# js43o/HifiDiff

Hardware: AMD Instinct MI355X
Metric: faces/sec (whole node), 16→128 1000-step reverse diffusion, batch 64 (higher is better)
Workload: dtype bf16

## Files before the change

hifidiff_amd/_lib.py:

```python
import ctypes
import os
import subprocess

import torch

_HERE = os.path.dirname(os.path.abspath(__file__))
LIB_PATH = os.path.join(_HERE, "libhifidiff_hip.so")
UNITS = [os.path.join(_HERE, "csrc", f) for f in ("hd_lib.hip", "hd_aux.hip", "hd_stages.hip", "hd_stages_rows.hip", "hd_strip.hip", "hd_dispatch_ln.hip", "hd_dispatch_lnface.hip", "hd_dispatch_bf16.hip", "hd_dispatch_misc.hip", "hd_lpips.hip", "hd_photo.hip", "hd_image.hip")]
SOURCES = UNITS + [os.path.join(_HERE, "csrc", f) for f in ("hd_gemm.hpp", "hd_dispatch.hpp", "hd_kernels.hpp", "hd_chain.hpp", "hd_conv.hpp", "hd_cr.hpp", "hd_vae.hpp", "hd_internal.hpp", "hd_faceset.hpp", "hd_stage_api.hpp", "hd_xcd.hpp", "hd_xcd2.hpp", "hd_face.hpp", "hd_strip.hpp", "hd_wide.hpp", "hd_end.hpp", "hd_color.hpp", "hd_metrics.hpp", "hd_lpips.hpp", "hd_photo.hpp", "hd_args.hpp", "hd_bicubic.hpp")]
HEADER = os.path.join(os.path.dirname(_HERE), "include", "hifidiff_hip.h")


def unit_deps(unit):
    import re
    seen, todo = [], [unit]
    while todo:
        f = os.path.normpath(todo.pop())
        if f in seen or not os.path.exists(f):
            continue
        seen.append(f)
        with open(f) as fh:
            for inc in re.findall(r'^\s*#include\s+"([^"]+)"', fh.read(), flags=re.M):
                todo.append(os.path.join(os.path.dirname(f), inc))
    return seen
# ... 33 lines not shown
class GemmNote(ctypes.Structure):
    _fields_ = [(n, ctypes.c_int32) for n in ("op_info", "family", "rows", "pair", "wk", "cpw", "nt", "wide_form", "threads", "grid_x", "grid_y")]


GEMM_DRY_RUN = 1


class ConvDesc(ctypes.Structure):
    _fields_ = [(n, ctypes.c_int32) for n in ("M", "C", "side", "face0", "stats_np", "stats_cnt", "film_off", "film_face_stride")] + \
               [("T1_elems", ctypes.c_int64)] + \
               [(n, ctypes.c_void_p) for n in ("X", "out", "out16", "stats_out", "stats_in", "film", "G", "pooled", "pooled16", "T1")]


class ConvNote(ctypes.Structure):
    _fields_ = [(n, ctypes.c_int32) for n in ("form", "centre_only", "C", "side", "bm", "mt", "ks", "nt", "strip", "depth", "faces_per_wg", "threads",
                                              "grid_x", "grid_y", "remap", "hint", "dw_path")] + [("gemm", GemmNote)]


CONV_HCA, CONV_DOWN, CONV_DWGATE = 0, 1, 2


def build(force=False, verbose=False):
    if not force and os.path.exists(LIB_PATH):
        newest = max(os.path.getmtime(p) for p in SOURCES + [HEADER])
        if os.path.getmtime(LIB_PATH) >= newest:
            return LIB_PATH
    hipcc = os.environ.get("HIPCC", "/opt/rocm/bin/hipcc")
    flags = ["--offload-arch=gfx950", "-O3", "-std=c++17", "-fPIC", "-Wno-unused-result", "-Wno-unused-function"]
    objdir = os.path.join(_HERE, "csrc", "build")
    os.makedirs(objdir, exist_ok=True)
    objs = [os.path.join(objdir, os.path.splitext(os.path.basename(u))[0] + ".o") for u in UNITS]
# ... 110 lines not shown
```

hifidiff_amd/csrc/hd_conv.hpp:

```cpp
#pragma once
#include "hd_gemm.hpp"
#ifndef HD_CONV_DEPTH
#define HD_CONV_DEPTH 8
#endif
#ifndef HD_CONV_NT_MINC
#define HD_CONV_NT_MINC 1024
#endif

#define HD_CONV_XCD_REMAP(C, grid_x, grid_y) ((C) >= 1024 && ((grid_y) & 7) == 0 && (grid_x) > 1)

namespace hd {

struct ConvP {
    int M;
    const unsigned short* X;
    const uint4* W;
    const float* bias;
    float* out;
    unsigned short* out16;
};

template <int C_, int S_, int BM_, int MT_, int KS_, int DEPTH_ = 8, bool STRIP_ = false, int NT_ = 1>
struct ConvCfg {
    static constexpr int C = C_, S = S_, HW = S_ * S_, BM = BM_, MT = MT_, KS = KS_, NT = NT_;
    static constexpr bool STRIP = STRIP_;
    static constexpr int RG = BM / (32 * MT);
    static constexpr int WAVES = RG * KS, THREADS = 64 * WAVES;
    static constexpr int NP = STRIP ? BM + 2 * S : (BM > HW ? BM : HW);
    static constexpr int ROWB = C * 2 + 16;
    static constexpr int KSTEPS = 9 * C / 16;
    static constexpr int SPT = C / 16, CPW = SPT / KS;
    static constexpr int NSTEP = 9 * CPW;
    static constexpr int XIN = (NP + 1) * ROWB;
    static constexpr int RED = KS > 1 ? KS * BM * 32 * 4 : 0;
// ... 1 lines not shown
    static constexpr int DEPTH = DEPTH_;
    static constexpr int OCC = (NT_ > 1 && C_ == 512) ? 4 : 1;
    static_assert(WAVES == 8 || WAVES == 4, "4 or 8 waves");
    static_assert(NSTEP >= DEPTH, "prefetch ring longer than the loop");
    static_assert(SPT % KS == 0 && BM % (32 * MT) == 0, "shape");
    static_assert((HW >= BM && HW % BM == 0) || (BM % HW == 0), "row tiles are whole faces or a face is whole row tiles");
    static_assert(!STRIP || (BM % S == 0 && HW % BM == 0 && HW > BM), "a strip is whole image rows of one face");
};

template <class K>
__global__ __launch_bounds__((K::THREADS), (K::OCC)) void hca_conv_kernel(const ConvP p) {
    extern __shared__ __attribute__((aligned(16))) char smem[];
    constexpr int C = K::C, S = K::S, HW = K::HW, MT = K::MT, KS = K::KS;
    const int tid = threadIdx.x, lane = tid & 63, wave = tid >> 6;
    const int rg = wave / KS, ksl = wave - rg * KS;
    int bx = blockIdx.x, tile = blockIdx.y;
    if (HD_CONV_XCD_REMAP(K::C, gridDim.x, gridDim.y)) {
        const int lin = blockIdx.y * gridDim.x + blockIdx.x, j = lin >> 3;
        bx = j % (int)gridDim.x;
        tile = (j / (int)gridDim.x) * 8 + (lin & 7);
    }
    const int row0 = bx * K::BM;
    const int pix0 = K::STRIP ? row0 - S : (row0 / K::NP) * K::NP;
    uint4 bq[K::DEPTH][K::NT];
    const uint4* Wl = p.W + ((size_t)tile * K::NT * K::KSTEPS + ksl * K::CPW) * 64 + lane;
#define HD_CONV_B(n, t) (K::C >= HD_CONV_NT_MINC ? nt_load_u4(&Wl[(size_t)((t) * K::KSTEPS + ((n) / K::CPW) * K::SPT + ((n) % K::CPW)) * 64]) \
                                      : Wl[(size_t)((t) * K::KSTEPS + ((n) / K::CPW) * K::SPT + ((n) % K::CPW)) * 64])
#pragma unroll
    for (int d = 0; d < K::DEPTH; ++d)
#pragma unroll
// ... 35 lines not shown
            for (int t = 0; t < 9; ++t) {
                const int yy = y + t / 3 - 1, xx = x + t % 3 - 1;
                const bool in = yy >= 0 && yy < S && xx >= 0 && xx < S;
                src_off[mt][t] = (in ? (sbase + yy * S + xx) : K::NP) * K::ROWB + h * 16;
            }
        }
    }
    f32x16_t acc[MT][K::NT];
#pragma unroll
    for (int mt = 0; mt < MT; ++mt)
#pragma unroll
        for (int t = 0; t < K::NT; ++t)
#pragma unroll
            for (int i = 0; i < 16; ++i) acc[mt][t][i] = 0.f;
    __syncthreads();

    const int cbase = ksl * K::CPW * 32;
#pragma unroll
    for (int n = 0; n < K::NSTEP; ++n) {
        const int tap = n / K::CPW, j = n % K::CPW;
        bf16x8_t a[MT];
#pragma unroll
        for (int mt = 0; mt < MT; ++mt) a[mt] = *reinterpret_cast<const bf16x8_t*>(smem + src_off[mt][tap] + cbase + j * 32);
#pragma unroll
        for (int t = 0; t < K::NT; ++t) {
            const bf16x8_t b = __builtin_bit_cast(bf16x8_t, bq[n % K::DEPTH][t]);
#pragma unroll
            for (int mt = 0; mt < MT; ++mt) acc[mt][t] = __builtin_amdgcn_mfma_f32_32x32x16_bf16(a[mt], b, acc[mt][t], 0, 0, 0);
        }
        if (n + K::DEPTH < K::NSTEP) {
#pragma unroll
            for (int t = 0; t < K::NT; ++t) bq[n % K::DEPTH][t] = HD_CONV_B(n + K::DEPTH, t);
            asm volatile("" ::: "memory");
        }
    }
#undef HD_CONV_B

    if constexpr (KS > 1) __syncthreads();
#pragma unroll
    for (int t = 0; t < K::NT; ++t) {
        const int col = (tile * K::NT + t) * 32 + (lane & 31);
        const float bias = p.bias[col];
        if constexpr (KS > 1) {
            float* red = reinterpret_cast<float*>(smem);
            if (t > 0) __syncthreads();
#pragma unroll
            for (int mt = 0; mt < MT; ++mt)
#pragma unroll
                for (int i = 0; i < 16; ++i) {
                    const int r = (rg * MT + mt) * 32 + (i & 3) + 8 * (i >> 2) + 4 * (lane >> 5);
                    red[(ksl * K::BM + r) * 32 + (lane & 31)] = acc[mt][t][i];
                }
            __syncthreads();
            for (int e = tid; e < K::BM * 32; e += K::THREADS) {
                float v = bias;
#pragma unroll
                for (int s = 0; s < KS; ++s) v += red[s * K::BM * 32 + e];
                v = fmaxf(v, 0.f);
                const int row = row0 + (e >> 5);
                if (row < p.M) {
                    p.out[(size_t)row * C + col] = v;
                    if (p.out16) p.out16[(size_t)row * C + col] = f32_to_bf16_bits(v);
                }
            }
        } else {
#pragma unroll
            for (int mt = 0; mt < MT; ++mt)
#pragma unroll
                for (int i = 0; i < 16; ++i) {
                    const int row = row0 + (rg * MT + mt) * 32 + (i & 3) + 8 * (i >> 2) + 4 * (lane >> 5);
                    const float v = fmaxf(acc[mt][t][i] + bias, 0.f);
                    if (row < p.M) {
                        p.out[(size_t)row * C + col] = v;
                        if (p.out16) p.out16[(size_t)row * C + col] = f32_to_bf16_bits(v);
                    }
                }
        }
    }
}

struct ConvLaunchNote { int C, S, BM, MT, KS, NT, strip, depth, threads, grid_x, grid_y, remap; };
inline thread_local ConvLaunchNote g_conv_note = {};

template <class K>
inline hipError_t launch_hca_conv(const ConvP& p, hipStream_t s) {
    if (K::SMEM > 65536) {
        static std::atomic<unsigned long long> granted{0};
        { const hipError_t e = grant_dynamic_lds(reinterpret_cast<const void*>(&hca_conv_kernel<K>), K::SMEM, granted); if (e != hipSuccess) return e; }
    }
    const dim3 grid((p.M + K::BM - 1) / K::BM, K::C / (32 * K::NT));
    g_conv_note = ConvLaunchNote{K::C, K::S, K::BM, K::MT, K::KS, K::NT, K::STRIP ? 1 : 0, K::DEPTH, K::THREADS, (int)grid.x, (int)grid.y,
                                 HD_CONV_XCD_REMAP(K::C, grid.x, grid.y) ? 1 : 0};
    hipLaunchKernelGGL((hca_conv_kernel<K>), grid, dim3(K::THREADS), K::SMEM, s, p);
    return hipGetLastError();
}

typedef ConvCfg<128, 16, 256, 2, 2, HD_CONV_DEPTH> ConvL0;
typedef ConvCfg<256, 8, 128, 2, 4, HD_CONV_DEPTH> ConvL1;
typedef ConvCfg<512, 4, 64, 2, 8, HD_CONV_DEPTH> ConvL2;
typedef ConvCfg<1024, 2, 32, 1, 8, 16> ConvL3;
#ifndef HD_CONV_L2X32_NT
#define HD_CONV_L2X32_NT 1
#endif
typedef ConvCfg<128, 32, 256, 2, 2, 4, true, 4> ConvL0x32;
typedef ConvCfg<256, 16, 256, 2, 2, 8, false, 2> ConvL1x32;
typedef ConvCfg<512, 8, 64, 2, 8, (HD_CONV_L2X32_NT > 1 ? 4 : 8), false, HD_CONV_L2X32_NT> ConvL2x32;
typedef ConvCfg<1024, 4, 64, 2, 8, 8, false, 2> ConvL3x32;
typedef ConvCfg<2048, 2, 32, 1, 8, 8, false, 2> ConvL4x32;

}
```

hifidiff_amd/csrc/hd_internal.hpp:

```cpp
#pragma once
#include <hip/hip_runtime.h>

#include <cmath>
#include <cstdio>
#include <cstring>
#include <functional>
#include <map>
#include <memory>
#include <string>
#include <unordered_map>
#include <vector>

#include "../../include/hifidiff_hip.h"
#include "hd_chain.hpp"
#include "hd_conv.hpp"
#include "hd_cr.hpp"
#include "hd_dispatch.hpp"
#include "hd_gemm.hpp"
#include "hd_kernels.hpp"
#include "hd_end.hpp"
#include "hd_faceset.hpp"
#include "hd_vae.hpp"
#include "hd_stage_api.hpp"

// ... 20 lines not shown

struct BlockW {
    std::string name;
    int C = 0, film_off = -1;
    PackedW conv1, conv3, sca, conv4, conv5;
    const float *dw_w = nullptr, *dw_b = nullptr, *beta = nullptr, *gamma = nullptr;
    const float* dw_wT = nullptr;
};

struct HcaW {
    int C = 0;
    PackedW mlp0, mlp2, sp0, fused;
    const float* sp3_w = nullptr;
    float sp3_b = 0.f;
    bool centre_only = false;
};

struct ResConv { PackedW w; int cin, cout, k, stride, pad; };
struct ResBlock { ResConv c1, c2, c3, ds; bool has_ds = false; };


struct Op {
    std::string name;
    std::function<hipError_t(hipStream_t)> run;
    std::shared_ptr<GemmP> gemm;
    bool skinny_affine = false;
    const void* out = nullptr;
    size_t out_elems = 0;
    int out_bf16 = 0;
    int lk = -1, ek = -1, mode = -1;
// ... 37 lines not shown
    float *id_emb = nullptr, *pool_tmp = nullptr, *mlp_tmp = nullptr, *sp_tmp = nullptr;
    unsigned short* res_buf[4] = {};
    uint4* face8 = nullptr;
    std::vector<Op> program;
    std::vector<Op> prep_program;
    StepState* step_state = nullptr;
    float* film_cur = nullptr;
    hipStream_t stream = nullptr;
    hipEvent_t done = nullptr;
    hipGraphExec_t graph_exec = nullptr;
    hipGraphExec_t graph_multi = nullptr;
    hipGraphExec_t graph_rows_exec = nullptr, graph_rows_multi = nullptr;
    unsigned rows_gen = 0;
    const float* rows_film = nullptr;
    bool fold_intro = false, fold_down0 = false, fold_up = false, fuse_end = false;
};

constexpr int kGraphSteps = 10;

struct VaeWs { float *X = nullptr, *T = nullptr, *S = nullptr, *mom = nullptr, *Q = nullptr, *K = nullptr, *V = nullptr, *resz = nullptr, *out3 = nullptr;
               unsigned short *H = nullptr, *H2 = nullptr, *Xb = nullptr, *U = nullptr; uint4* in8 = nullptr; double* part = nullptr; int B = 0, R = 0; };

struct LpScale { float shift[3], scale[3]; };
struct LpWs { uint4* in8 = nullptr; unsigned short *f[5] = {}, *pool[2] = {}; double* part = nullptr; int B = 0, R = 0; };

struct ProgramKey {
    const void* ptr[6] = {};
    uint64_t flags = 0, seed = 0;
    bool operator==(const ProgramKey& o) const { return memcmp(ptr, o.ptr, sizeof(ptr)) == 0 && flags == o.flags && seed == o.seed; }
};
// ... 164 lines not shown
    bool xcd_ok = false;
    bool xcd_on = true;
    int xcd2_mask = 0;
    bool xcd2_on = true;
    int xcd_phase_limit = 0, xcd_force_global = 0;
    struct FStage { unsigned* sync = nullptr; float* pool_part = nullptr; };
    std::map<int, FStage> fstages;
    bool face_ok = false;
    bool face_on = true;
    int face_block_limit = 0;
    bool end_fold = true;
    bool end_fused = true;
    bool up_fold = true;
    bool down_fold = true;
    bool intro_fold = true;
    int face_l1_rows = 16;
    int stage_limit_first = -1;
    unsigned* xcd_tmo_host = nullptr;
    unsigned* xcd_tmo_dev = nullptr;
    unsigned* abort_dev = nullptr;
    int stage_test_abort = 0;

    int op_limit = -1, prep_limit = -1;

    bool profiling = false;
    hipEvent_t ev0 = nullptr, ev1 = nullptr;
    double last_loop_ms = 0.0;
    int last_steps = 0;
    std::map<std::string, std::pair<void*, std::pair<size_t, int>>> dbg;
    std::map<std::string, PackedW> dbg_packed;
// ... 324 lines not shown
            if (!o.bn.empty()) v = v * s[n] + off[n];
            bf[n] = v;
        }
        if (o.S2 > 1) {
            std::vector<float> bp(N);
            const int cg = N / o.S2;
            for (int np = 0; np < N; ++np) bp[np] = bf[(np % cg) * o.S2 + np / cg];
            bf.swap(bp);
        }
        rc = upload_vec(c, bf, &out->bias);
        if (rc) return rc;
    }
    return HD_OK;
}

bool dwgate_ok(int hw) { return hw == 1 || hw == 4 || hw == 16 || hw == 64 || hw == 256; }

hipError_t dispatch_gemm(const GemmP& p, LdKind lk, EpKind ek, int mode, hipStream_t s) {
    if (lk == LK_LN) return p.film_face_stride != 0 ? dispatch_gemm_ln_face(p, ek, mode, s) : dispatch_gemm_ln_shared(p, ek, mode, s);
    if (lk == LK_BF16 || lk == LK_BF16S) return dispatch_gemm_bf16(p, lk, ek, mode, s);
    return dispatch_gemm_misc(p, lk, ek, mode, s);
}

int choose_mode(const GemmP& p, bool pair) {
    const int ncols = pair ? p.N / 2 : p.N;
    const int nb64 = (ncols + 63) / 64, nb32 = (ncols + 31) / 32;
    static const int force = hd_env("HD_GEMM_MODE") ? atoi(hd_env("HD_GEMM_MODE")) : -1;
    if (force >= 0) return force;
    const int nb256 = (ncols + (pair ? 127 : 255)) / (pair ? 128 : 256);
    if (p.Kp <= 256 && nb256 <= 2 && ((p.M + 31) / 32) * nb256 >= 512) return 4;
// ... 236 lines not shown
    p.out = dst.X; p.ldo = dst.C; p.stats_out = dst.sx; p.out16 = dst.Xb;
    add_gemm(c, prog, name, p, LK_CONV_BF16, EK_BIASF32, dst.M >= 4096 ? 3 : -1);
}

void add_up(hd_ctx* c, std::vector<Op>& prog, const std::string& name, const PackedW& w, const void* in, bool in_bf16, int M_in,
            int H_in, int C_in, float* out, const float* skip, int r, unsigned short* out16 = nullptr, float2* stats = nullptr) {
    GemmP p = base_gemm(w, M_in);
    p.A = in; p.lda = C_in; p.Hin = H_in; p.Win = H_in; p.shuffle_r = r;
    p.out = out; p.ldo = w.N / (r * r); p.resid = skip; p.bias = nullptr;
    p.out16 = out16; p.stats_out = stats;
    const int hint = M_in >= 4096 ? 3 : (M_in >= 1024 && M_in < 2048 && w.Kp >= 1024) ? 1 : -1;
    add_gemm(c, prog, name, p, in_bf16 ? LK_BF16 : LK_F32, EK_PIXSHUF, hint);
}

void add_hca(hd_ctx* c, std::vector<Op>& prog, const std::string& name, const HcaW& hw, const unsigned short* in, float* out,
             unsigned short* out16, int M, int H) {
    static const bool no_lds = hd_env("HD_NO_CONVLDS") != nullptr;
    if (!hw.centre_only && !no_lds) {
        ConvP q{};
        q.M = M; q.X = in; q.W = hw.fused.w; q.bias = hw.fused.bias; q.out = out; q.out16 = out16;
        const int C = hw.C;
        int which = -1;
        if (C == 128 && H == 16) which = 0; else if (C == 256 && H == 8) which = 1; else if (C == 512 && H == 4) which = 2;
        else if (C == 1024 && H == 2) which = 3; else if (C == 256 && H == 16) which = 4; else if (C == 512 && H == 8) which = 5;
        else if (C == 1024 && H == 4) which = 6; else if (C == 2048 && H == 2) which = 7; else if (C == 128 && H == 32) which = 8;
        if (which >= 0) {
            Op op;
            op.name = name; op.out = out; op.out_elems = (size_t)M * C;
            op.run = [q, which](hipStream_t s) -> hipError_t {
                switch (which) {
                    case 0: return launch_hca_conv<ConvL0>(q, s);
                    case 1: return launch_hca_conv<ConvL1>(q, s);
                    case 2: return launch_hca_conv<ConvL2>(q, s);
                    case 3: return launch_hca_conv<ConvL3>(q, s);
                    case 4: return launch_hca_conv<ConvL1x32>(q, s);
                    case 5: return launch_hca_conv<ConvL2x32>(q, s);
                    case 6: return launch_hca_conv<ConvL3x32>(q, s);
                    case 8: return launch_hca_conv<ConvL0x32>(q, s);
                    default: return launch_hca_conv<ConvL4x32>(q, s);
                }
            };
            prog.push_back(op);
            return;
        }
// ... 68 lines not shown
```

hifidiff_amd/csrc/hd_lib.hip:

```cpp
#include "hd_internal.hpp"

static std::string g_create_error;
void set_contextless_error(const std::string& msg) { g_create_error = msg; }

namespace {

int alloc_chain(hd_ctx* c, Chain& ch) {
    const int L = c->L, B = ch.B;
    const bool names = (ch.index == 0);
    auto& dbg = c->ws->dbg;
    int rc = 0;
    for (int l = 0; l < 5; ++l) {
        Level& v = ch.lv[l];
        v.C = WIDTH << l; v.H = L >> l; v.M = B * v.H * v.H;
        const size_t mc = (size_t)v.M * v.C;
        rc |= alloc_level(c, v, B, mc, names, l);
        const int pi = 4 - l;
        rc |= ws_alloc(c, &ch.prior[pi], mc); rc |= ws_alloc(c, &ch.gate_c[pi], (size_t)B * v.C);
        rc |= ws_alloc(c, &ch.gate_s[pi], (size_t)v.M);
        if (rc) return rc;
        if (names) {
            const std::string ps = std::to_string(pi);
            dbg["Xg" + std::to_string(l)] = {v.Xg, {mc, 1}};
            dbg["prior" + ps] = {ch.prior[pi], {mc, 0}}; dbg["wc" + ps] = {ch.gate_c[pi], {(size_t)B * v.C, 0}};
// ... 180 lines not shown
                const hipError_t e = mode_is_rows(c->mode) ? run_face_rows_stage(c128 ? 128 : 256, c128 ? 32 : c->face_l1_rows, r, s)
                                                           : run_face_stage(c128 ? 128 : 256, c128 ? 32 : c->face_l1_rows, r, s);
                if (e == hipSuccess) { ++c->stage_count; ++c->face_stage_count; return e; }
                (void)hipGetLastError();
                c->face_on = false;
            }
            if (intro_first) { const hipError_t e = intro_first(s); if (e != hipSuccess) return e; }
            for (auto& o : *sub) { const hipError_t e = o.run(s); if (e != hipSuccess) return e; }
            return hipSuccess;
        };
        prog.push_back(op);
        np = lv.C / 32; cnt = 32;
    };
    const bool fold_down0 = fold_intro && c->down_fold && c->face_l1_rows == 16 && c->ch->lv[1].C == 256 && c->ch->lv[1].H == 8 && c->den_down[0].K == 512 && c->den_down[0].N == 256;
    chp->fold_intro = fold_intro; chp->fold_down0 = fold_down0;
    std::vector<Op> down0;
    for (int l = 0; l < 4; ++l) {
        if (l >= 2) add_stage(enc[l], c->ch->lv[l], nullptr);
        else add_face_stage(enc[l], c->ch->lv[l], nullptr, true, l == 0 && fold_intro, (l == 1 && fold_down0) ? &down0[0] : nullptr);
        if (stage_rc) return stage_rc;
        add_down(c, (l == 0 && fold_down0) ? down0 : prog, "downs." + std::to_string(l), c->den_down[l], c->ch->lv[l], c->ch->lv[l + 1]);
        np = c->ch->lv[l + 1].C / 32; cnt = 32;
    }
    const bool cond = c->conditional;
    for (int j = 0; j < 8; ++j) {
        GateOut g0; g0.gate_c = c->ch->gate_c[0]; g0.gate_s = c->ch->gate_s[0]; g0.add = c->ch->idc_term;
        add_naf_block(c, prog, c->den_blocks[bi++], c->ch->lv[4], nullptr, &np, &cnt, (cond && j == 7) ? &g0 : nullptr);
    }
    if (cond) add_hca(c, prog, "hcas.0", c->hca[0], c->ch->lv[4].Xg, c->ch->lv[4].Y, c->ch->lv[4].Yb, c->ch->lv[4].M, c->ch->lv[4].H);
    const bool fuse_end = cond && fold_intro && c->end_fold && L == 16 && c->ch->lv[0].C == 128 && c->ch->lv[0].H == 16 && !c->hca[4].centre_only;
// ... 3 lines not shown
        const int l = 3 - i;
        const Level &hi = c->ch->lv[l + 1], &lo = c->ch->lv[l];
        const bool fold_up = i == 3 && fold_intro && c->up_fold && lo.C == 128 && lo.H == 16 && c->den_up[3].K == 256 && c->den_up[3].N == 512;
        std::vector<Op> up3;
        if (i == 3) chp->fold_up = fold_up;
        add_up(c, fold_up ? up3 : prog, "ups." + std::to_string(i), c->den_up[i], cond ? hi.Yb : hi.Xb, true, hi.M, hi.H, hi.C, lo.X, lo.X, 2, lo.Xb, lo.sx);
        np = lo.C / 32; cnt = 32;
        GateOut g; g.gate_c = c->ch->gate_c[i + 1]; g.gate_s = c->ch->gate_s[i + 1];
        if (l >= 2) {
            add_stage(2, lo, cond ? &g : nullptr);
            if (stage_rc) return stage_rc;
        } else {
            add_face_stage(2, lo, cond ? &g : nullptr, !cond, false, nullptr, fold_up ? &up3[0] : nullptr, cond ? hi.Yb : hi.Xb);
            if (stage_rc) return stage_rc;
        }
        if (cond) add_hca(c, (i == 3 && fuse_end) ? hca4 : prog, "hcas." + std::to_string(i + 1), c->hca[i + 1], lo.Xg, lo.Y, i < 3 ? lo.Yb : nullptr, lo.M, lo.H);
    }
    {
        const float *X = cond ? c->ch->lv[0].Y : c->ch->lv[0].X, *w = c->ending_wT, *b = eb->dev; float* eps = c->ch->eps;
        const int M = c->ch->lv[0].M;
        Chain* chp = c->ch;
        EndP ep{};
        std::function<hipError_t(hipStream_t)> hca4_run;
        if (fuse_end) {
            ep.B = B; ep.Xg = c->ch->lv[0].Xg; ep.W = c->hca[4].fused.w; ep.bias = c->hca[4].fused.bias; ep.ewT = w; ep.eb = b; ep.eps = eps;
            hca4_run = hca4[0].run;
        }
        auto sched_args = [c, chp, L]() {
            SchedArgs sa{};
            if (!mode_is_loop(c->mode)) return sa;
            const size_t per_face = (size_t)4 * L * L;
// ... 190 lines not shown
    hipLaunchKernelGGL(time_embed_kernel, dim3((n * 64 + 255) / 256), dim3(256), 0, s, t_dev, c->freq_dev, c->temb_a, n);
    hipLaunchKernelGGL((linear_f32_kernel<false>), dim3(1024 / 64, (n + 63) / 64), dim3(256), 0, s, c->temb_a, 128, w1->dev, b1->dev, c->temb_b, 1024, n, 1024, 128);
    hipLaunchKernelGGL((linear_f32_kernel<true>), dim3(512 / 64, (n + 63) / 64), dim3(256), 0, s, c->temb_b, 1024, w3->dev, b3->dev, c->temb_c, 512, n, 512, 512);
    hipLaunchKernelGGL((linear_f32_kernel<true>), dim3((c->film_total + 63) / 64, (n + 63) / 64), dim3(256), 0, s, c->temb_c, 512, c->film_W, c->film_b,
                       c->film_table, c->film_total, n, c->film_total, FILM_IN);
    hipLaunchKernelGGL(film_fold_kernel, dim3(2048 / 256, (unsigned)c->den_blocks.size(), n), dim3(256), 0, s, c->film_table, c->ln_pack, c->film_blocks_dev, c->film_total);
    HIPCHECK(c, hipGetLastError());
    return HD_OK;
}



int setup_xcd(hd_ctx* c) {
    c->xcd_ok = false; c->face_ok = false;
    c->end_fold = getenv("HD_NO_END_FOLD") == nullptr;
    if (c->S != 1 || getenv("HD_NO_XCD")) return HD_OK;
    hipDeviceProp_t prop;
    if (hipGetDeviceProperties(&prop, c->device) != hipSuccess || prop.multiProcessorCount != XS_GROUPS * XS_GROUP_WG) return HD_OK;
    HIPCHECK(c, hipHostMalloc(reinterpret_cast<void**>(&c->xcd_tmo_host), 64, hipHostMallocMapped));
    c->xcd_tmo_host[0] = 0;
    HIPCHECK(c, hipHostGetDevicePointer(reinterpret_cast<void**>(&c->xcd_tmo_dev), c->xcd_tmo_host, 0));
    if (int rc = dev_alloc(c, &c->abort_dev, 64)) return rc;
    HIPCHECK(c, hipMemset(c->abort_dev, 0, 64 * sizeof(unsigned)));
    c->xcd_ok = true;
    c->xcd2_mask = getenv("HD_XCD2") ? (atoi(getenv("HD_XCD2")) & 3) : 1;
    c->face_ok = getenv("HD_NO_FACE") == nullptr;
    c->intro_fold = getenv("HD_NO_INTRO_FOLD") == nullptr;
    c->down_fold = getenv("HD_NO_DOWN_FOLD") == nullptr;
    c->up_fold = getenv("HD_NO_UP_FOLD") == nullptr;
    if (const char* e = getenv("HD_FACE_L1_ROWS")) c->face_l1_rows = atoi(e) == 32 ? 32 : 16;
// ... 235 lines not shown
        rc |= pack_weight(c, "denoiser.downs." + std::to_string(i), &c->den_down[i]);
        { PackOpts o; o.S2 = 4; rc |= pack_weight(c, "denoiser.ups." + std::to_string(i) + ".0", &c->den_up[i], o); }
        if (c->conditional) rc |= pack_weight(c, "fpg.downs." + std::to_string(i), &c->fpg_down[i]);
    }
    for (int i = 0; i < 5 && c->conditional; ++i) { PackOpts o; o.S2 = i ? 4 : 1; rc |= pack_weight(c, "fpg.convs." + std::to_string(i) + ".0", &c->fpg_convs[i], o); }
    if (c->conditional) { PackOpts o; o.S2 = c->S * c->S; rc |= pack_weight(c, "denoiser.idc_conv", &c->idc_conv, o); }
    if (rc) return rc;
    for (int i = 0; i < 5 && c->conditional; ++i) {
        HcaW& h = c->hca[i];
        const std::string p = "denoiser.hcas." + std::to_string(i);
        h.C = (WIDTH << 4) >> i;
        h.centre_only = ((c->L >> (4 - i)) == 1);
        rc |= pack_weight(c, p + ".channel_mlp.0", &h.mlp0); rc |= pack_weight(c, p + ".channel_mlp.2", &h.mlp2);
        { PackOpts o; o.bn = p + ".spatial_mlp.1"; rc |= pack_weight(c, p + ".spatial_mlp.0", &h.sp0, o); }
        { PackOpts o; o.bn = p + ".fused_mlp.1"; o.centre_only = h.centre_only; rc |= pack_weight(c, p + ".fused_mlp.0", &h.fused, o); }
        if (rc) return rc;
        std::vector<float> s, o2;
        rc = bn_affine(c, p + ".spatial_mlp.4", s, o2);
        if (rc) return rc;
        const RawTensor *w3 = find_raw(c, p + ".spatial_mlp.3.weight"), *b3 = find_raw(c, p + ".spatial_mlp.3.bias");
        std::vector<float> wf(w3->numel);
        for (size_t k = 0; k < w3->numel; ++k) wf[k] = w3->host[k] * s[0];
        h.sp3_b = b3->host[0] * s[0] + o2[0];
        rc = upload_vec(c, wf, &h.sp3_w);
        if (rc) return rc;
    }
    auto load_res = [&](const std::string& conv, const std::string& bn, int cin, int cout, int k, int stride, int pad, ResConv& r) -> int {
        PackOpts o; o.bn = bn;
        if (cin == 3) o.cin_pad = 8;
        r.cin = cin; r.cout = cout; r.k = k; r.stride = stride; r.pad = pad;
// ... 1275 lines not shown
        o.centre_only = centre;
        if (const int rc = pack_weight(c, name, &pw, o)) return rc;
        HIPCHECK(c, hipDeviceSynchronize());
        it = c->dbg_packed.emplace(key, pw).first;
    }
    std::vector<Op> prog;
    if (down) {
        Level src{}, dst{};
        src.C = C; src.H = side; src.M = d->M; src.Xb = const_cast<unsigned short*>(static_cast<const unsigned short*>(d->X));
        dst.C = N; dst.H = side / 2; dst.M = d->M / 4; dst.X = d->out; dst.Xb = static_cast<unsigned short*>(d->out16);
        dst.sx = reinterpret_cast<float2*>(d->stats_out);
        add_down(c, prog, "debug_conv." + name, it->second, src, dst);
    } else {
        HcaW hw;
        hw.C = C; hw.fused = it->second; hw.centre_only = centre;
        add_hca(c, prog, "debug_conv." + name, hw, static_cast<const unsigned short*>(d->X), d->out, static_cast<unsigned short*>(d->out16), d->M, side);
    }
    note->centre_only = centre ? 1 : 0;
    note->hint = prog[0].hint;
    note->gemm.op_info = op_info_word(prog[0]);
    if (flags & HD_GEMM_DRY_RUN) return HD_OK;
    g_launch_note = LaunchNote{};
    g_conv_note = ConvLaunchNote{};
    if (const int rc = run_ops(c, prog, static_cast<hipStream_t>(stream))) return rc;
    if (prog[0].gemm) {
        const LaunchNote& ln = g_launch_note;
        hd_gemm_note& g = note->gemm;
        note->form = 2;
        g.family = ln.family; g.rows = ln.rows; g.pair = ln.pair; g.wk = ln.wk; g.cpw = ln.cpw; g.nt = ln.nt;
        g.wide_form = ln.wide_form; g.threads = ln.threads; g.grid_x = ln.grid_x; g.grid_y = ln.grid_y;
        note->threads = ln.threads; note->grid_x = ln.grid_x; note->grid_y = ln.grid_y;
    } else {
        const ConvLaunchNote& cn = g_conv_note;
        note->form = 1;
        note->C = cn.C; note->side = cn.S; note->bm = cn.BM; note->mt = cn.MT; note->ks = cn.KS; note->nt = cn.NT; note->strip = cn.strip;
        note->depth = cn.depth; note->faces_per_wg = (!cn.strip && cn.BM > cn.S * cn.S) ? cn.BM / (cn.S * cn.S) : 1;
        note->threads = cn.threads; note->grid_x = cn.grid_x; note->grid_y = cn.grid_y; note->remap = cn.remap;
    }
    return HD_OK;
}
static int64_t read_to_host(hd_ctx* c, const void* dev, size_t n, int is_bf16, float* host_out, int64_t max_elems) {
    if (!host_out) return (int64_t)n;
    if ((int64_t)n > max_elems) HD_FAIL(c, HD_ERR_INVALID, "debug read needs %zu elements", n);
    HIPCHECK(c, hipSetDevice(c->device));
    HIPCHECK(c, hipDeviceSynchronize());
    if (is_bf16) {
        std::vector<unsigned short> tmp(n);
        HIPCHECK(c, hipMemcpy(tmp.data(), dev, n * 2, hipMemcpyDeviceToHost));
        for (size_t i = 0; i < n; ++i) { unsigned u = (unsigned)tmp[i] << 16; memcpy(&host_out[i], &u, 4); }
    } else {
        HIPCHECK(c, hipMemcpy(host_out, dev, n * sizeof(float), hipMemcpyDeviceToHost));
    }
// ... 56 lines not shown
        HIPCHECK(c, hipMemcpy(e->first, tmp.data(), n * 2, hipMemcpyHostToDevice));
    } else {
        HIPCHECK(c, hipMemcpy(e->first, host_in, n * sizeof(float), hipMemcpyHostToDevice));
    }
    return HD_OK;
}

int hd_set_option(hd_ctx* c, const char* key, int value) {
    if (!c || !key) return HD_ERR_INVALID;
    const std::string k = key;
    if (k == "xcd") c->xcd_on = value != 0;
    else if (k == "xcd2") c->xcd2_on = value != 0;
    else if (k == "xcd_phase_limit") c->xcd_phase_limit = value;
    else if (k == "xcd_force_global") c->xcd_force_global = value;
    else if (k == "face") c->face_on = value != 0;
    else if (k == "face_block_limit") c->face_block_limit = value;
    else if (k == "stage_limit_first") c->stage_limit_first = value;
    else if (k == "stage_test_abort") c->stage_test_abort = value;
    else HD_FAIL(c, HD_ERR_INVALID, "unknown option %s", key);
    invalidate_step_graphs(c);
    return HD_OK;
}
int hd_get_option(hd_ctx* c, const char* key) {
    if (!c || !key) return HD_ERR_INVALID;
    const std::string k = key;
    if (k == "xcd") return (c->xcd_ok && c->xcd_on) ? 1 : 0;
    if (k == "xcd2") return (c->xcd_ok && c->xcd_on && c->xcd2_on) ? c->xcd2_mask : 0;
    if (k == "xcd_stages") return (int)c->xstages.size();
    if (k == "face_stages") return (int)c->fstages.size();
    if (k == "face_l1_rows") return c->face_l1_rows;
// ... 1 lines not shown
    if (k == "sample_face_stage_launches") return c->sample_face_stages;
    if (k == "rows_stage_launches") return c->rows_stages;
    if (k == "masked_faces") return c->mask.faces.valid_for(c->ws->B) ? c->mask.faces.count() : 0;
    if (k == "preview") return c->preview.on ? 1 : 0;
    if (k == "guide") return c->guide.on ? 1 : 0;
    if (k == "guided_faces") return c->guide.faces.valid_for(c->ws->B) ? c->guide.faces.count() : 0;
    if (k == "pool_capacity") return c->pool_cap;
    if (k == "pool_valid") { int n = 0; for (char v : c->pool_ok) n += v != 0; return n; }
    if (k == "graph_captures") return c->graph_captures;
    const Chain* ch = c->ws->chains.empty() ? nullptr : &c->ws->chains[0];
    const bool face_runs = c->xcd_ok && c->face_on && c->ws->chains.size() == 1;
    if (k == "intro_fold") return (ch && ch->fold_intro && face_runs) ? 1 : 0;
    if (k == "down_fold") return (ch && ch->fold_down0 && face_runs) ? 1 : 0;
    if (k == "up_fold") return (ch && ch->fold_up && face_runs) ? 1 : 0;
    if (k == "end_fold") return (ch && ch->fuse_end && c->end_fused) ? 1 : 0;
    return HD_ERR_INVALID;
}

int hd_check(hd_ctx* c) {
    if (!c) return HD_ERR_INVALID;
    return check_xcd(c);
}

int hd_set_profiling(hd_ctx* c, int on) { if (!c) return HD_ERR_INVALID; c->profiling = on != 0; return HD_OK; }

int hd_get_profile(hd_ctx* c, double* loop_ms, double* step_ms_avg, int64_t* weight_bytes_per_step, double* flops_per_face_step) {
    if (!c) return HD_ERR_INVALID;
    float ms = 0.f;
    if (c->profiling && c->last_steps > 0) {
        HIPCHECK(c, hipEventSynchronize(c->ev1));
// ... 11 lines not shown
```

include/hifidiff_hip.h:

```cpp
#ifndef HIFIDIFF_HIP_H
#define HIFIDIFF_HIP_H

#include <stddef.h>
#include <stdint.h>

#ifdef __cplusplus
extern "C" {
#endif

typedef struct hd_ctx hd_ctx;

enum hd_status {
    HD_OK = 0,
    HD_ERR_INVALID = -1,
    HD_ERR_HIP = -2,
    HD_ERR_WEIGHTS = -3,
    HD_ERR_NOT_READY = -4
};

typedef struct hd_tensor_desc {
    const char* name;
    const void* data;
    int32_t ndim;
    int64_t shape[4];
// ... 149 lines not shown
    void* G;
    float* pooled;
    void* pooled16;
    float* T1;
} hd_conv_desc;
typedef struct hd_conv_note {
    int32_t form;
    int32_t centre_only;
    int32_t C, side;
    int32_t bm, mt, ks, nt, strip, depth;
    int32_t faces_per_wg;
    int32_t threads, grid_x, grid_y;
    int32_t remap;
    int32_t hint;
    int32_t dw_path;
    hd_gemm_note gemm;
} hd_conv_note;
enum { HD_CONV_HCA = 0, HD_CONV_DOWN = 1, HD_CONV_DWGATE = 2 };
int hd_debug_conv(hd_ctx* ctx, int kind, const char* weight, const char* weight2, const hd_conv_desc* desc, int flags, hd_conv_note* note,
                  void* stream);
int hd_set_option(hd_ctx* ctx, const char* key, int value);
int hd_get_option(hd_ctx* ctx, const char* key);
int hd_check(hd_ctx* ctx);
int hd_set_profiling(hd_ctx* ctx, int on);
int hd_get_profile(hd_ctx* ctx, double* loop_ms, double* step_ms_avg, int64_t* weight_bytes_per_step,
                   double* flops_per_face_step);

#ifdef __cplusplus
}
#endif
// ... 2 lines not shown
```

Baseline: 66.94.

## Add 16-column MFMA 3x3 conv kernel for C=1024 side-2 HCA layer

Adds a conv kernel using 16x16x32 bf16 MFMA tiles with 16 output columns per workgroup and an 8-way K split, plus a matching weight packer. It is used for the C=1024, 2x2 HCA fused conv when the batch exactly fills the tile (default hca_tiles=1). Narrower column tiles give more workgroups for this small spatial layer, improving CU occupancy, at the cost of an extra packed weight copy and a cross-wave LDS reduction. Stamp instrumentation hooks and note fields are also added.

```diff
diff --git a/hifidiff_amd/_lib.py b/hifidiff_amd/_lib.py
--- a/hifidiff_amd/_lib.py
+++ b/hifidiff_amd/_lib.py
@@ -71,7 +71,7 @@
 
 class ConvNote(ctypes.Structure):
     _fields_ = [(n, ctypes.c_int32) for n in ("form", "centre_only", "C", "side", "bm", "mt", "ks", "nt", "strip", "depth", "faces_per_wg", "threads",
-                                              "grid_x", "grid_y", "remap", "hint", "dw_path")] + [("gemm", GemmNote)]
+                                              "grid_x", "grid_y", "remap", "hint", "dw_path", "cols")] + [("gemm", GemmNote)]
 
 
 CONV_HCA, CONV_DOWN, CONV_DWGATE = 0, 1, 2
diff --git a/hifidiff_amd/csrc/hd_conv.hpp b/hifidiff_amd/csrc/hd_conv.hpp
--- a/hifidiff_amd/csrc/hd_conv.hpp
+++ b/hifidiff_amd/csrc/hd_conv.hpp
@@ -18,6 +18,9 @@
     const float* bias;
     float* out;
     unsigned short* out16;
+#ifdef HD_STAMPS
+    unsigned long long* stamps;
+#endif
 };
 
 template <int C_, int S_, int BM_, int MT_, int KS_, int DEPTH_ = 8, bool STRIP_ = false, int NT_ = 1>
@@ -49,6 +52,7 @@
     constexpr int C = K::C, S = K::S, HW = K::HW, MT = K::MT, KS = K::KS;
     const int tid = threadIdx.x, lane = tid & 63, wave = tid >> 6;
     const int rg = wave / KS, ksl = wave - rg * KS;
+    HD_STAMP(0);
     int bx = blockIdx.x, tile = blockIdx.y;
     if (HD_CONV_XCD_REMAP(K::C, gridDim.x, gridDim.y)) {
         const int lin = blockIdx.y * gridDim.x + blockIdx.x, j = lin >> 3;
@@ -114,6 +118,7 @@
 #pragma unroll
             for (int i = 0; i < 16; ++i) acc[mt][t][i] = 0.f;
     __syncthreads();
+    HD_STAMP(1);
 
     const int cbase = ksl * K::CPW * 32;
 #pragma unroll
@@ -128,6 +133,7 @@
 #pragma unroll
             for (int mt = 0; mt < MT; ++mt) acc[mt][t] = __builtin_amdgcn_mfma_f32_32x32x16_bf16(a[mt], b, acc[mt][t], 0, 0, 0);
         }
+        if (n == 0) HD_STAMP(2);
         if (n + K::DEPTH < K::NSTEP) {
 #pragma unroll
             for (int t = 0; t < K::NT; ++t) bq[n % K::DEPTH][t] = HD_CONV_B(n + K::DEPTH, t);
@@ -136,6 +142,7 @@
     }
 #undef HD_CONV_B
 
+    HD_STAMP(3);
     if constexpr (KS > 1) __syncthreads();
 #pragma unroll
     for (int t = 0; t < K::NT; ++t) {
@@ -152,6 +159,7 @@
                     red[(ksl * K::BM + r) * 32 + (lane & 31)] = acc[mt][t][i];
                 }
             __syncthreads();
+            if (t == 0) HD_STAMP(4);
             for (int e = tid; e < K::BM * 32; e += K::THREADS) {
                 float v = bias;
 #pragma unroll
@@ -177,9 +185,10 @@
                 }
         }
     }
-}
-
-struct ConvLaunchNote { int C, S, BM, MT, KS, NT, strip, depth, threads, grid_x, grid_y, remap; };
+    HD_STAMP(5);
+}
+
+struct ConvLaunchNote { int C, S, BM, MT, KS, NT, strip, depth, threads, grid_x, grid_y, remap, cols; };
 inline thread_local ConvLaunchNote g_conv_note = {};
 
 template <class K>
@@ -190,7 +199,7 @@
     }
     const dim3 grid((p.M + K::BM - 1) / K::BM, K::C / (32 * K::NT));
     g_conv_note = ConvLaunchNote{K::C, K::S, K::BM, K::MT, K::KS, K::NT, K::STRIP ? 1 : 0, K::DEPTH, K::THREADS, (int)grid.x, (int)grid.y,
-                                 HD_CONV_XCD_REMAP(K::C, grid.x, grid.y) ? 1 : 0};
+                                 HD_CONV_XCD_REMAP(K::C, grid.x, grid.y) ? 1 : 0, 32};
     hipLaunchKernelGGL((hca_conv_kernel<K>), grid, dim3(K::THREADS), K::SMEM, s, p);
     return hipGetLastError();
 }
@@ -208,4 +217,163 @@
 typedef ConvCfg<1024, 4, 64, 2, 8, 8, false, 2> ConvL3x32;
 typedef ConvCfg<2048, 2, 32, 1, 8, 8, false, 2> ConvL4x32;
 
-}
+template <int C_, int S_, int BM_, int DEPTH_>
+struct Conv16Cfg {
+    static constexpr int C = C_, S = S_, HW = S_ * S_, BM = BM_, MT = BM_ / 16, KS = 8;
+    static constexpr int WAVES = 8, THREADS = 512;
+    static constexpr int NP = BM;
+    static constexpr int ROWB = C * 2 + 16;
+    static constexpr int KSTEPS = 9 * C / 32;
+    static constexpr int SPT = C / 32, CPW = SPT / KS;
+    static constexpr int NSTEP = 9 * CPW;
+    static constexpr int XIN = (NP + 1) * ROWB;
+    static constexpr int RED = KS * BM * 16 * 4;
+    static constexpr int SMEM = XIN > RED ? XIN : RED;
+    static constexpr int DEPTH = DEPTH_;
+    static_assert(BM % HW == 0 && BM % 16 == 0 && SPT % KS == 0 && NSTEP >= DEPTH, "shape");
+    static_assert(SMEM <= 160 * 1024, "LDS of a gfx950 compute unit");
+};
+
+typedef __attribute__((ext_vector_type(4))) float f32x4_t;
+
+template <class K>
+__global__ __launch_bounds__(512, 1) void hca_conv16_kernel(const ConvP p) {
+    extern __shared__ __attribute__((aligned(16))) char smem[];
+    constexpr int C = K::C, S = K::S, HW = K::HW, MT = K::MT, KS = K::KS;
+    const int tid = threadIdx.x, lane = tid & 63, ksl = tid >> 6;
+    HD_STAMP(0);
+    int bx = blockIdx.x, tile = blockIdx.y;
+    if (gridDim.x > 1) {
+        const int lin = blockIdx.y * gridDim.x + blockIdx.x, j = lin >> 3;
+        bx = j % (int)gridDim.x;
+        tile = (j / (int)gridDim.x) * 8 + (lin & 7);
+    }
+    const int row0 = bx * K::BM;
+    uint4 bq[K::DEPTH];
+    const uint4* Wl = p.W + ((size_t)tile * K::KSTEPS + ksl * K::CPW) * 64 + lane;
+#define HD_CONV16_B(n) (K::C >= HD_CONV_NT_MINC ? nt_load_u4(&Wl[(size_t)(((n) / K::CPW) * K::SPT + ((n) % K::CPW)) * 64]) \
+                                        : Wl[(size_t)(((n) / K::CPW) * K::SPT + ((n) % K::CPW)) * 64])
+#pragma unroll
+    for (int d = 0; d < K::DEPTH; ++d) bq[d] = HD_CONV16_B(d);
+    const int col = tile * 16 + (tid & 15);
+    const float bias = p.bias[col];
+
+    {
+        constexpr int PPR = C / 8;
+        const uint4* src = reinterpret_cast<const uint4*>(p.X) + (long long)row0 * PPR;
+        constexpr int NIT = K::NP * PPR / K::THREADS;
+        static_assert(K::NP * PPR % K::THREADS == 0 && NIT <= 16, "staging registers");
+        uint4 stage[NIT];
+        const int last = (p.M - row0) * PPR - 1;
+#pragma unroll
+        for (int it = 0; it < NIT; ++it) {
+            const int i = tid + it * K::THREADS;
+            stage[it] = src[i > last ? last : i];
+        }
+#pragma unroll
+        for (int it = 0; it < NIT; ++it) {
+            const int i = tid + it * K::THREADS;
+            const int px = i / PPR, q = i - px * PPR;
+            *reinterpret_cast<uint4*>(smem + px * K::ROWB + q * 16) = i <= last ? stage[it] : make_uint4(0, 0, 0, 0);
+        }
+        for (int i = tid; i < K::ROWB / 16; i += K::THREADS) *reinterpret_cast<uint4*>(smem + K::NP * K::ROWB + i * 16) = make_uint4(0, 0, 0, 0);
+    }
+    int src_off[MT][9];
+    {
+        const int r = lane & 15, q = lane >> 4;
+#pragma unroll
+        for (int mt = 0; mt < MT; ++mt) {
+            const int pl = mt * 16 + r;
+            const int f = pl / HW, rem = pl - f * HW, y = rem / S, x = rem - y * S;
+#pragma unroll
+            for (int t = 0; t < 9; ++t) {
+                const int yy = y + t / 3 - 1, xx = x + t % 3 - 1;
+                const bool in = yy >= 0 && yy < S && xx >= 0 && xx < S;
+                src_off[mt][t] = (in ? (f * HW + yy * S + xx) : K::NP) * K::ROWB + q * 16;
+            }
+        }
+    }
+    f32x4_t acc[MT];
+#pragma unroll
+    for (int mt = 0; mt < MT; ++mt)
+#pragma unroll
+        for (int i = 0; i < 4; ++i) acc[mt][i] = 0.f;
+    __syncthreads();
+    HD_STAMP(1);
+
+    const int cbase = ksl * K::CPW * 64;
+#pragma unroll
+    for (int n = 0; n < K::NSTEP; ++n) {
+        const int tap = n / K::CPW, j = n % K::CPW;
+        bf16x8_t a[MT];
+#pragma unroll
+        for (int mt = 0; mt < MT; ++mt) a[mt] = *reinterpret_cast<const bf16x8_t*>(smem + src_off[mt][tap] + cbase + j * 64);
+        const bf16x8_t b = __builtin_bit_cast(bf16x8_t, bq[n % K::DEPTH]);
+#pragma unroll
+        for (int mt = 0; mt < MT; ++mt) acc[mt] = __builtin_amdgcn_mfma_f32_16x16x32_bf16(a[mt], b, acc[mt], 0, 0, 0);
+        if (n == 0) HD_STAMP(2);
+        if (n + K::DEPTH < K::NSTEP) {
+            bq[n % K::DEPTH] = HD_CONV16_B(n + K::DEPTH);
+            asm volatile("" ::: "memory");
+        }
+    }
+#undef HD_CONV16_B
+    HD_STAMP(3);
+
+    __syncthreads();
+    float* red = reinterpret_cast<float*>(smem);
+#pragma unroll
+    for (int mt = 0; mt < MT; ++mt)
+#pragma unroll
+        for (int i = 0; i < 4; ++i) red[(ksl * K::BM + mt * 16 + 4 * (lane >> 4) + i) * 16 + (lane & 15)] = acc[mt][i];
+    __syncthreads();
+    HD_STAMP(4);
+#pragma unroll
+    for (int e = tid; e < K::BM * 16; e += K::THREADS) {
+        float v = bias;
+#pragma unroll
+        for (int s = 0; s < KS; ++s) v += red[s * K::BM * 16 + e];
+        v = fmaxf(v, 0.f);
+        const int row = row0 + (e >> 4);
+        if (row < p.M) {
+            p.out[(size_t)row * C + col] = v;
+            if (p.out16) p.out16[(size_t)row * C + col] = f32_to_bf16_bits(v);
+        }
+    }
+    HD_STAMP(5);
+}
+
+static __global__ void pack_conv16_kernel(const float* __restrict__ src, uint4* __restrict__ dst, int N, int C, const float* __restrict__ nscale) {
+    const int ksteps = 9 * C / 32;
+    const size_t total = (size_t)(N >> 4) * ksteps * 64;
+    for (size_t e = (size_t)blockIdx.x * blockDim.x + threadIdx.x; e < total; e += (size_t)gridDim.x * blockDim.x) {
+        const int lane = (int)(e & 63);
+        const size_t tk = e >> 6;
+        const int ks = (int)(tk % ksteps), nt = (int)(tk / ksteps);
+        const int n = nt * 16 + (lane & 15);
+        float v[8];
+#pragma unroll
+        for (int j = 0; j < 8; ++j) {
+            const int k = ks * 32 + 8 * (lane >> 4) + j;
+            const int tap = k / C, c = k - tap * C;
+            float x = src[((size_t)n * C + c) * 9 + tap];
+            if (nscale) x *= nscale[n];
+            v[j] = x;
+        }
+        dst[e] = pack8(v);
+    }
+}
+
+template <class K>
+inline hipError_t launch_hca_conv16(const ConvP& p, hipStream_t s) {
+    static std::atomic<unsigned long long> granted{0};
+    { const hipError_t e = grant_dynamic_lds(reinterpret_cast<const void*>(&hca_conv16_kernel<K>), K::SMEM, granted); if (e != hipSuccess) return e; }
+    const dim3 grid((p.M + K::BM - 1) / K::BM, K::C / 16);
+    g_conv_note = ConvLaunchNote{K::C, K::S, K::BM, K::MT, K::KS, 0, 0, K::DEPTH, K::THREADS, (int)grid.x, (int)grid.y, grid.x > 1 ? 1 : 0, 16};
+    hipLaunchKernelGGL((hca_conv16_kernel<K>), grid, dim3(K::THREADS), K::SMEM, s, p);
+    return hipGetLastError();
+}
+
+typedef Conv16Cfg<1024, 2, 64, 16> Conv16L3;
+
+}
diff --git a/hifidiff_amd/csrc/hd_internal.hpp b/hifidiff_amd/csrc/hd_internal.hpp
--- a/hifidiff_amd/csrc/hd_internal.hpp
+++ b/hifidiff_amd/csrc/hd_internal.hpp
@@ -58,6 +58,7 @@
     const float* sp3_w = nullptr;
     float sp3_b = 0.f;
     bool centre_only = false;
+    const uint4* w16 = nullptr;
 };
 
 struct ResConv { PackedW w; int cin, cout, k, stride, pad; };
@@ -125,6 +126,7 @@
     unsigned rows_gen = 0;
     const float* rows_film = nullptr;
     bool fold_intro = false, fold_down0 = false, fold_up = false, fuse_end = false;
+    int hca16_have = 0, hca16_fit = 0;
 };
 
 constexpr int kGraphSteps = 10;
@@ -319,6 +321,7 @@
     bool up_fold = true;
     bool down_fold = true;
     bool intro_fold = true;
+    int hca_tiles = 1;
     int face_l1_rows = 16;
     int stage_limit_first = -1;
     unsigned* xcd_tmo_host = nullptr;
@@ -673,6 +676,29 @@
     return HD_OK;
 }
 
+int pack_hca16(hd_ctx* c, const std::string& name, const std::string& bn, const uint4** out) {
+    const RawTensor* w = find_raw(c, name + ".weight");
+    if (!w || w->shape.size() != 4 || w->shape[0] != w->shape[1] || w->shape[2] != 3 || w->shape[3] != 3 || w->shape[0] % 32 != 0)
+        HD_FAIL(c, HD_ERR_WEIGHTS, "missing %s.weight, or not a [C][C][3][3] conv", name.c_str());
+    const int C = (int)w->shape[0];
+    const float* nscale = nullptr;
+    if (!bn.empty()) {
+        std::vector<float> s, off;
+        int rc = bn_affine(c, bn, s, off);
+        if (rc) return rc;
+        rc = upload_vec(c, s, &nscale);
+        if (rc) return rc;
+    }
+    const size_t n16 = (size_t)(C / 16) * (9 * C / 32) * 64;
+    uint4* dst = nullptr;
+    if (const int rc = dev_alloc(c, &dst, n16)) return rc;
+    hipLaunchKernelGGL(pack_conv16_kernel, dim3((unsigned)std::min<size_t>((n16 + 255) / 256, 65535)), dim3(256), 0, 0, w->dev, dst, C, C, nscale);
+    HIPCHECK(c, hipGetLastError());
+    *out = dst;
+    return HD_OK;
+}
+inline bool hca16_shape(int C, int H) { return C == 1024 && H == 2; }
+
 bool dwgate_ok(int hw) { return hw == 1 || hw == 4 || hw == 16 || hw == 64 || hw == 256; }
 
 hipError_t dispatch_gemm(const GemmP& p, LdKind lk, EpKind ek, int mode, hipStream_t s) {
@@ -939,7 +965,7 @@
 }
 
 void add_hca(hd_ctx* c, std::vector<Op>& prog, const std::string& name, const HcaW& hw, const unsigned short* in, float* out,
-             unsigned short* out16, int M, int H) {
+             unsigned short* out16, int M, int H, int* tiles16 = nullptr) {
     static const bool no_lds = hd_env("HD_NO_CONVLDS") != nullptr;
     if (!hw.centre_only && !no_lds) {
         ConvP q{};
@@ -952,7 +978,14 @@
         if (which >= 0) {
             Op op;
             op.name = name; op.out = out; op.out_elems = (size_t)M * C;
-            op.run = [q, which](hipStream_t s) -> hipError_t {
+            ConvP q16 = q;
+            q16.W = hca16_shape(C, H) ? hw.w16 : nullptr;
+            const bool fits = q16.W != nullptr && M == 64 * H * H;
+            if (tiles16) *tiles16 = q16.W ? (fits ? 3 : 1) : 0;
+            const hd_ctx* cc = c;
+            op.run = [q, q16, which, fits, cc](hipStream_t s) -> hipError_t {
+                if (q16.W && (cc->hca_tiles == 2 || (cc->hca_tiles == 1 && fits)))
+                    return launch_hca_conv16<Conv16L3>(q16, s);
                 switch (which) {
                     case 0: return launch_hca_conv<ConvL0>(q, s);
                     case 1: return launch_hca_conv<ConvL1>(q, s);
diff --git a/hifidiff_amd/csrc/hd_lib.hip b/hifidiff_amd/csrc/hd_lib.hip
--- a/hifidiff_amd/csrc/hd_lib.hip
+++ b/hifidiff_amd/csrc/hd_lib.hip
@@ -218,6 +218,7 @@
     };
     const bool fold_down0 = fold_intro && c->down_fold && c->face_l1_rows == 16 && c->ch->lv[1].C == 256 && c->ch->lv[1].H == 8 && c->den_down[0].K == 512 && c->den_down[0].N == 256;
     chp->fold_intro = fold_intro; chp->fold_down0 = fold_down0;
+    chp->hca16_have = 0; chp->hca16_fit = 0;
     std::vector<Op> down0;
     for (int l = 0; l < 4; ++l) {
         if (l >= 2) add_stage(enc[l], c->ch->lv[l], nullptr);
@@ -251,7 +252,9 @@
             add_face_stage(2, lo, cond ? &g : nullptr, !cond, false, nullptr, fold_up ? &up3[0] : nullptr, cond ? hi.Yb : hi.Xb);
             if (stage_rc) return stage_rc;
         }
-        if (cond) add_hca(c, (i == 3 && fuse_end) ? hca4 : prog, "hcas." + std::to_string(i + 1), c->hca[i + 1], lo.Xg, lo.Y, i < 3 ? lo.Yb : nullptr, lo.M, lo.H);
+        int t16 = 0;
+        if (cond) add_hca(c, (i == 3 && fuse_end) ? hca4 : prog, "hcas." + std::to_string(i + 1), c->hca[i + 1], lo.Xg, lo.Y, i < 3 ? lo.Yb : nullptr, lo.M, lo.H, &t16);
+        chp->hca16_have |= (t16 & 1) << (i + 1); chp->hca16_fit |= (t16 >> 1) << (i + 1);
     }
     {
         const float *X = cond ? c->ch->lv[0].Y : c->ch->lv[0].X, *w = c->ending_wT, *b = eb->dev; float* eps = c->ch->eps;
@@ -472,6 +475,7 @@
 int setup_xcd(hd_ctx* c) {
     c->xcd_ok = false; c->face_ok = false;
     c->end_fold = getenv("HD_NO_END_FOLD") == nullptr;
+    if (const char* e = hd_env("HD_HCA_TILES")) c->hca_tiles = std::min(std::max(atoi(e), 0), 2);
     if (c->S != 1 || getenv("HD_NO_XCD")) return HD_OK;
     hipDeviceProp_t prop;
     if (hipGetDeviceProperties(&prop, c->device) != hipSuccess || prop.multiProcessorCount != XS_GROUPS * XS_GROUP_WG) return HD_OK;
@@ -737,6 +741,8 @@
         rc |= pack_weight(c, p + ".channel_mlp.0", &h.mlp0); rc |= pack_weight(c, p + ".channel_mlp.2", &h.mlp2);
         { PackOpts o; o.bn = p + ".spatial_mlp.1"; rc |= pack_weight(c, p + ".spatial_mlp.0", &h.sp0, o); }
         { PackOpts o; o.bn = p + ".fused_mlp.1"; o.centre_only = h.centre_only; rc |= pack_weight(c, p + ".fused_mlp.0", &h.fused, o); }
+        if (rc) return rc;
+        if (hca16_shape(h.C, c->L >> (4 - i))) rc = pack_hca16(c, p + ".fused_mlp.0", p + ".fused_mlp.1", &h.w16);
         if (rc) return rc;
         std::vector<float> s, o2;
         rc = bn_affine(c, p + ".spatial_mlp.4", s, o2);
@@ -2042,6 +2048,18 @@
     } else {
         HcaW hw;
         hw.C = C; hw.fused = it->second; hw.centre_only = centre;
+        if (hca16_shape(C, side) && c->hca_tiles != 0) {
+            auto i16 = c->dbg_packed.find(name + "#conv16");
+            if (i16 == c->dbg_packed.end()) {
+                PackedW pw;
+                const uint4* w16 = nullptr;
+                if (const int rc = pack_hca16(c, name, "", &w16)) return rc;
+                HIPCHECK(c, hipDeviceSynchronize());
+                pw.w = const_cast<uint4*>(w16);
+                i16 = c->dbg_packed.emplace(name + "#conv16", pw).first;
+            }
+            hw.w16 = i16->second.w;
+        }
         add_hca(c, prog, "debug_conv." + name, hw, static_cast<const unsigned short*>(d->X), d->out, static_cast<unsigned short*>(d->out16), d->M, side);
     }
     note->centre_only = centre ? 1 : 0;
@@ -2063,7 +2081,7 @@
         note->form = 1;
         note->C = cn.C; note->side = cn.S; note->bm = cn.BM; note->mt = cn.MT; note->ks = cn.KS; note->nt = cn.NT; note->strip = cn.strip;
         note->depth = cn.depth; note->faces_per_wg = (!cn.strip && cn.BM > cn.S * cn.S) ? cn.BM / (cn.S * cn.S) : 1;
-        note->threads = cn.threads; note->grid_x = cn.grid_x; note->grid_y = cn.grid_y; note->remap = cn.remap;
+        note->threads = cn.threads; note->grid_x = cn.grid_x; note->grid_y = cn.grid_y; note->remap = cn.remap; note->cols = cn.cols;
     }
     return HD_OK;
 }
@@ -2150,6 +2168,7 @@
     else if (k == "xcd_phase_limit") c->xcd_phase_limit = value;
     else if (k == "xcd_force_global") c->xcd_force_global = value;
     else if (k == "face") c->face_on = value != 0;
+    else if (k == "hca_tiles") { if (value < 0 || value > 2) HD_FAIL(c, HD_ERR_INVALID, "hca_tiles = %d (0, 1 or 2)", value); c->hca_tiles = value; }
     else if (k == "face_block_limit") c->face_block_limit = value;
     else if (k == "stage_limit_first") c->stage_limit_first = value;
     else if (k == "stage_test_abort") c->stage_test_abort = value;
@@ -2181,6 +2200,7 @@
     if (k == "down_fold") return (ch && ch->fold_down0 && face_runs) ? 1 : 0;
     if (k == "up_fold") return (ch && ch->fold_up && face_runs) ? 1 : 0;
     if (k == "end_fold") return (ch && ch->fuse_end && c->end_fused) ? 1 : 0;
+    if (k == "hca_tiles") return !ch ? 0 : c->hca_tiles == 2 ? ch->hca16_have : c->hca_tiles == 1 ? ch->hca16_fit : 0;
     return HD_ERR_INVALID;
 }
 
diff --git a/include/hifidiff_hip.h b/include/hifidiff_hip.h
--- a/include/hifidiff_hip.h
+++ b/include/hifidiff_hip.h
@@ -187,6 +187,7 @@
     int32_t remap;
     int32_t hint;
     int32_t dw_path;
+    int32_t cols;
     hd_gemm_note gemm;
 } hd_conv_note;
 enum { HD_CONV_HCA = 0, HD_CONV_DOWN = 1, HD_CONV_DWGATE = 2 };
```

New measurement: 66.22. 0.989x the previous value.
